# interstellar/zkvm

Hardware: AMD Instinct MI355X
Metric: ZkVM tx verifications/sec (batch) (higher is better)
Workload: dtype u32 limb pairs of radix-2^51 (v_mad_u64_u32)

## Files before the change

zkvm_amd/csrc/kernels.hpp:

```cpp
#pragma once
#include "curve.hpp"
#include "quad.hpp"
#include "sc_dev.hpp"

namespace zk {

constexpr uint32_t ENTRY_NEG = 1u << 31;
constexpr uint32_t ENTRY_DYN = 1u << 30;
constexpr uint32_t ENTRY_IDX = (1u << 30) - 1;
constexpr int NIELS_WORDS = 32;
constexpr int EXT_WORDS = 40;
constexpr int REDUCE_CHUNK = 64;
#ifndef ZK_REDUCE_CHUNK_BIG
#define ZK_REDUCE_CHUNK_BIG 16
#endif
constexpr int REDUCE_CHUNK_BIG = ZK_REDUCE_CHUNK_BIG;
constexpr int TABLE_WORDS = 24;
constexpr int TABLE_STRIDE = 32;

struct JobDesc {
  const uint32_t* dyn_scalars;
  const uint64_t* dyn_offsets;
  uint64_t n_dyn;
  const uint32_t* st_scalars;
  const uint32_t* st_index;
  const uint64_t* st_offsets;
  uint64_t n_static;
  uint32_t n_msm;
  int w;
  int n_windows;
  uint32_t n_buckets;
};


__device__ __forceinline__ void load_niels(ge_niels& q, const uint32_t* row) {
  const uint4* r4 = reinterpret_cast<const uint4*>(row);
  uint32_t w[32];
#pragma unroll
  for (int i = 0; i < 8; ++i) {
    uint4 v = r4[i];
    w[4 * i] = v.x; w[4 * i + 1] = v.y; w[4 * i + 2] = v.z; w[4 * i + 3] = v.w;
  }
#pragma unroll
  for (int i = 0; i < 10; ++i) { q.ypx.v[i] = w[i]; q.ymx.v[i] = w[10 + i]; q.xy2d.v[i] = w[20 + i]; }
}

__device__ __forceinline__ void store_niels(uint32_t* row, const ge_niels& q, uint32_t valid) {
  uint32_t w[32];
#pragma unroll
  for (int i = 0; i < 10; ++i) { w[i] = q.ypx.v[i]; w[10 + i] = q.ymx.v[i]; w[20 + i] = q.xy2d.v[i]; }
  w[30] = valid; w[31] = 0;
  uint4* r4 = reinterpret_cast<uint4*>(row);
#pragma unroll
  for (int i = 0; i < 8; ++i) r4[i] = make_uint4(w[4 * i], w[4 * i + 1], w[4 * i + 2], w[4 * i + 3]);
}

__device__ __forceinline__ void load_ext(ge& p, const uint32_t* row) {
  const uint4* r4 = reinterpret_cast<const uint4*>(row);
  uint32_t w[40];
#pragma unroll
  for (int i = 0; i < 10; ++i) {
    uint4 v = r4[i];
    w[4 * i] = v.x; w[4 * i + 1] = v.y; w[4 * i + 2] = v.z; w[4 * i + 3] = v.w;
  }
#pragma unroll
  for (int i = 0; i < 10; ++i) { p.X.v[i] = w[i]; p.Y.v[i] = w[10 + i]; p.Z.v[i] = w[20 + i]; p.T.v[i] = w[30 + i]; }
}

__device__ __forceinline__ void store_ext(uint32_t* row, const ge& p) {
  uint32_t w[40];
#pragma unroll
  for (int i = 0; i < 10; ++i) { w[i] = p.X.v[i]; w[10 + i] = p.Y.v[i]; w[20 + i] = p.Z.v[i]; w[30 + i] = p.T.v[i]; }
  uint4* r4 = reinterpret_cast<uint4*>(row);
#pragma unroll
  for (int i = 0; i < 10; ++i) r4[i] = make_uint4(w[4 * i], w[4 * i + 1], w[4 * i + 2], w[4 * i + 3]);
}

__device__ __forceinline__ void load_table_row(ge_niels& q, const uint32_t* row) {
  const uint4* r4 = reinterpret_cast<const uint4*>(row);
  uint32_t w[24];
#pragma unroll
  for (int i = 0; i < 6; ++i) {
    uint4 v = r4[i];
    w[4 * i] = v.x; w[4 * i + 1] = v.y; w[4 * i + 2] = v.z; w[4 * i + 3] = v.w;
  }
  fe_from_words(q.ypx, w);
  fe_from_words(q.ymx, w + 8);
  fe_from_words(q.xy2d, w + 16);
}

__device__ __forceinline__ void store_table_row(uint32_t* row, const ge_niels& q) {
  uint32_t w[24];
  fe_to_words(w, q.ypx);
  fe_to_words(w + 8, q.ymx);
  fe_to_words(w + 16, q.xy2d);
  uint4* r4 = reinterpret_cast<uint4*>(row);
#pragma unroll
  for (int i = 0; i < 6; ++i) r4[i] = make_uint4(w[4 * i], w[4 * i + 1], w[4 * i + 2], w[4 * i + 3]);
}

__device__ __forceinline__ uint32_t find_row(const uint64_t* __restrict__ offsets, uint32_t n_msm, uint64_t g) {
  uint32_t lo = 0, hi = n_msm;
  while (hi - lo > 1) {
    uint32_t mid = (lo + hi) >> 1;
    if (offsets[mid] <= g) lo = mid; else hi = mid;
  }
  return lo;
}

__global__ void __launch_bounds__(256)
k_decompress(const uint32_t* __restrict__ pts, uint32_t* __restrict__ rows, uint64_t n,
             const uint64_t* __restrict__ offsets, uint32_t n_msm, uint32_t* __restrict__ msm_fail,
             unsigned long long* __restrict__ bad_index, uint8_t* __restrict__ ok_out) {
  uint64_t i = (uint64_t)blockIdx.x * blockDim.x + threadIdx.x;
  if (i >= n) return;
  const uint4* p4 = reinterpret_cast<const uint4*>(pts + 8 * i);
  uint4 a = p4[0], b = p4[1];
  uint32_t w[8] = {a.x, a.y, a.z, a.w, b.x, b.y, b.z, b.w};
  fe x, y;
  bool ok = ristretto_decode_affine(x, y, w);
  ge_niels q;
  niels_from_affine(q, x, y);
  if (!ok) niels_identity(q);
  if (rows) store_niels(rows + NIELS_WORDS * i, q, ok ? 1u : 0u);
  if (ok_out) ok_out[i] = ok ? 1 : 0;
  if (!ok) {
    if (bad_index) atomicMin(bad_index, (unsigned long long)i);
    if (msm_fail) {
      uint32_t m = (n_msm > 1 && offsets) ? find_row(offsets, n_msm, i) : 0;
      atomicOr(&msm_fail[m], 1u);
    }
  }
}

struct DecodeRoutes {
  uint64_t n[4] = {0, 0, 0, 0};
  void note(bool split, uint64_t points) {
    n[split ? 2 : 0] += 1;
    n[split ? 3 : 1] += points;
  }
};

constexpr int DEC_WORDS = 64;

struct DecFront { fe s, u1, u2, v, w, w7; bool pre_ok; };
__device__ __forceinline__ void dec_front(DecFront& d, const uint32_t* __restrict__ pts, uint64_t i) {
  const uint4* p4 = reinterpret_cast<const uint4*>(pts + 8 * i);
  uint4 a = p4[0], b = p4[1];
  uint32_t w[8] = {a.x, a.y, a.z, a.w, b.x, b.y, b.z, b.w};
  fe ss, u2_sqr, t;
  fe_from_words(d.s, w);
  uint32_t chk[8];
  fe_to_words(chk, d.s);
  bool canonical = true;
#pragma unroll
  for (int k = 0; k < 8; ++k) canonical &= (chk[k] == w[k]);
// ... 872 lines not shown
    accept[m] = failed ? 0 : 1;
    return;
  }
  const bool ident = have ? ge_is_identity(acc) : true;
  accept[m] = (ident && !failed) ? 1 : 0;
}

__global__ void __launch_bounds__(64)
k_from_uniform(const uint32_t* __restrict__ in, uint32_t* __restrict__ out, uint64_t n) {
  const uint64_t i = (uint64_t)blockIdx.x * blockDim.x + threadIdx.x;
  if (i >= n) return;
  uint32_t w[16];
  const uint4* i4 = reinterpret_cast<const uint4*>(in + 16 * i);
#pragma unroll
  for (int k = 0; k < 4; ++k) { uint4 v = i4[k]; w[4 * k] = v.x; w[4 * k + 1] = v.y; w[4 * k + 2] = v.z; w[4 * k + 3] = v.w; }
  ge p;
  ristretto_from_uniform_words(p, w);
  uint32_t enc[8];
  ristretto_encode(enc, p);
  uint4* o = reinterpret_cast<uint4*>(out + 8 * i);
  o[0] = make_uint4(enc[0], enc[1], enc[2], enc[3]);
  o[1] = make_uint4(enc[4], enc[5], enc[6], enc[7]);
}

__global__ void __launch_bounds__(64)
k_spin(unsigned long long cycles, uint32_t* __restrict__ sink) {
  const unsigned long long t0 = clock64();
  unsigned long long spins = 0;
  while ((unsigned long long)clock64() - t0 < cycles) ++spins;
  if (sink && spins == ~0ull) *sink = 1;
}

__global__ void __launch_bounds__(256)
k_hbm_copy(const uint4* __restrict__ src, uint4* __restrict__ dst, uint64_t n_vec) {
  const uint64_t i = (uint64_t)blockIdx.x * 256 + threadIdx.x;
  if (i < n_vec) dst[i] = src[i];
}

__global__ void __launch_bounds__(256)
k_batch_init(uint32_t* __restrict__ status, uint32_t* __restrict__ msm_fail, uint32_t* __restrict__ wellformed,
             uint32_t n_msm) {
  const uint32_t i = blockIdx.x * blockDim.x + threadIdx.x;
  if (i < n_msm) {
    msm_fail[i] = 0;
    if (wellformed) wellformed[i] = 0xffffffffu;
  }
  if (i == 0) {
    status[0] = 0; status[1] = 0;
    status[2] = 0xffffffffu; status[3] = 0xffffffffu;
    status[8] = 0;
    status[9] = 0;
  }
}

__global__ void __launch_bounds__(256)
k_pack_bitmap(const uint8_t* __restrict__ accept, const uint32_t* __restrict__ wellformed ,
              uint8_t* __restrict__ bitmap, uint32_t n_msm) {
  const uint32_t byte = blockIdx.x * blockDim.x + threadIdx.x;
  if (byte >= (n_msm + 7) / 8) return;
  uint32_t v = 0;
#pragma unroll
  for (int k = 0; k < 8; ++k) {
    const uint32_t i = byte * 8 + k;
    if (i < n_msm && accept[i] && (!wellformed || wellformed[i])) v |= 1u << k;
  }
  bitmap[byte] = (uint8_t)v;
}


__global__ void __launch_bounds__(64)
k_tbl_base(const uint32_t* __restrict__ rows , uint32_t* __restrict__ base, uint32_t n_set, int w, int W) {
  const uint32_t j = blockIdx.x * blockDim.x + threadIdx.x;
  if (j >= n_set) return;
  ge_niels q;
  load_niels(q, rows + (uint64_t)j * NIELS_WORDS);
  ge p;
  ge_identity(p);
  ge_madd(p, p, q, false);
  for (int t = 0; t < W; ++t) {
    store_ext(base + ((uint64_t)t * n_set + j) * EXT_WORDS, p);
    if (t + 1 < W) {
      for (int k = 0; k < w - 1; ++k) ge_double<false>(p, p);
      ge_double<true>(p, p);
    }
  }
}

__global__ void __launch_bounds__(64)
k_tbl_multiples(const uint32_t* __restrict__ base, uint32_t* __restrict__ tmp, uint32_t* __restrict__ table,
                uint64_t n_lanes, uint32_t H) {
  const uint64_t lane = (uint64_t)blockIdx.x * blockDim.x + threadIdx.x;
  if (lane >= n_lanes) return;
  ge p, q;
  load_ext(p, base + lane * EXT_WORDS);
  q = p;
  fe prod = fe_one();
  uint32_t* mytmp = tmp + lane * (uint64_t)H * EXT_WORDS;
  for (uint32_t d = 0; d < H; ++d) {
    if (d) ge_add(q, q, p);
    fe_mul(prod, prod, q.Z);
    ge rec;
    rec.X = q.X; rec.Y = q.Y; rec.Z = q.Z; rec.T = prod;
    store_ext(mytmp + (uint64_t)d * EXT_WORDS, rec);
  }
  fe inv;
  fe_invert(inv, prod);
  uint32_t* myrows = table + lane * (uint64_t)H * TABLE_STRIDE;
  for (uint32_t d = H; d-- > 0;) {
    ge rec;
    load_ext(rec, mytmp + (uint64_t)d * EXT_WORDS);
    fe prev = fe_one();
    if (d) {
      ge r2;
      load_ext(r2, mytmp + (uint64_t)(d - 1) * EXT_WORDS);
      prev = r2.T;
    }
    fe zinv, x, y;
    fe_mul(zinv, inv, prev);
    fe_mul(inv, inv, rec.Z);
    fe_mul(x, rec.X, zinv);
    fe_mul(y, rec.Y, zinv);
    ge_niels nq;
    niels_from_affine(nq, x, y);
    store_table_row(myrows + (uint64_t)d * TABLE_STRIDE, nq);
  }
}

__global__ void __launch_bounds__(256)
k_static_digits(const uint32_t* __restrict__ st_scalars, int16_t* __restrict__ digits, uint64_t n_static, int w,
                int W, uint32_t* __restrict__ status, const uint32_t* __restrict__ row_map ,
                const uint32_t* __restrict__ n_active , uint32_t rows_per_msm, uint32_t fold_small_negatives) {
  uint64_t k = (uint64_t)blockIdx.x * blockDim.x + threadIdx.x;
  if (k >= n_static) return;
  if (row_map) {
    const uint32_t slot = (uint32_t)(k / rows_per_msm);
    if (slot >= *n_active) return;
    k = (uint64_t)row_map[slot] * rows_per_msm + k % rows_per_msm;
  }
  const uint32_t* sc = st_scalars + 8 * k;
  if (sc[7] >> 31) atomicOr(&status[0], 2u);
  for (int t = 0; t < W; ++t) digits[(uint64_t)t * n_static + k] = 0;
  if (fold_small_negatives) {
    const uint32_t l[8] = ZK_SC_L;
    uint32_t v[8];
    uint64_t br = 0;
    for (int i = 0; i < 8; ++i) { const uint64_t d = (uint64_t)l[i] - sc[i] - br; v[i] = (uint32_t)d; br = (d >> 32) & 1; }
    uint32_t high = v[0] >> 14;
    for (int i = 1; i < 8; ++i) high |= v[i];
    if (br == 0 && high == 0 && v[0] != 0 && w >= 15) { digits[k] = (int16_t)(-(int)v[0]); return; }
  }
  for_each_digit(sc, w, W, [&](int t, int d) { digits[(uint64_t)t * n_static + k] = (int16_t)d; });
}

template <bool kSkipZeros>
__global__ void __launch_bounds__(256)
k_static_accumulate(const int16_t* __restrict__ digits, const uint64_t* __restrict__ st_offsets,
                    const uint32_t* __restrict__ st_index, const uint32_t* __restrict__ table, uint32_t n_set,
                    uint32_t H, int W, int P, uint32_t n_msm, uint64_t n_static, uint32_t* __restrict__ partials,
                    const uint32_t* __restrict__ row_map ,
                    const uint32_t* __restrict__ n_active ,
                    uint32_t interleave ) {
  const uint64_t lane = (uint64_t)blockIdx.x * blockDim.x + threadIdx.x;
  if (lane >= (uint64_t)n_msm * W * P) return;
  const uint32_t part = (uint32_t)(lane % P);
  uint32_t slot = (uint32_t)((lane / P) % n_msm);
  const uint32_t t = (uint32_t)(lane / ((uint64_t)P * n_msm));
  if (n_active && slot >= *n_active) return;
  if (interleave > 1) { const uint32_t per = n_msm / interleave; slot = (slot % per) * interleave + slot / per; }
  const uint32_t tx = row_map ? row_map[slot] : slot;
  const uint64_t k0 = st_offsets[tx], k1 = st_offsets[tx + 1];
  const int16_t* dig = digits + (uint64_t)t * n_static;
  const uint64_t tbase = (uint64_t)t * n_set;
  ge acc;
  ge_identity(acc);
  auto fetch = [&](uint64_t k, ge_niels& q, bool& neg, bool& any) {
    int d = dig[k];
    d = (d == -32768) ? 32768 : d;
    any = d != 0;
    const uint32_t idx = st_index ? st_index[k] : (uint32_t)(k - k0);
    const uint32_t mag = (uint32_t)(d < 0 ? -d : d);
    if (!kSkipZeros || any) load_table_row(q, table + ((tbase + idx) * H + (mag ? mag - 1 : 0)) * TABLE_STRIDE);
    if (!any) niels_identity(q);
    neg = d < 0;
  };
  uint64_t k = k0 + part;
  ge_niels cur, nxt;
  bool cur_neg = false, nxt_neg = false, cur_any = false, nxt_any = false;
  if (k < k1) fetch(k, cur, cur_neg, cur_any);
  while (k < k1) {
    const uint64_t kn = k + P;
    if (kn < k1) fetch(kn, nxt, nxt_neg, nxt_any);
    if (!kSkipZeros || __any(cur_any)) ge_madd(acc, acc, cur, cur_neg);
    cur = nxt; cur_neg = nxt_neg; cur_any = nxt_any;
    k = kn;
  }
  store_ext(partials + (((uint64_t)slot * W + t) * P + part) * EXT_WORDS, acc);
}

__device__ inline void static_combine_slot(const uint32_t* __restrict__ partials, uint32_t n_partials, const uint32_t* __restrict__ dyn_sum,
                                           const uint8_t* __restrict__ dyn_ok, uint32_t slot, uint32_t tx, int lane,
                                           uint8_t* __restrict__ accept, uint32_t* __restrict__ out_points) {
  ge acc;
  ge_identity(acc);
  for (uint32_t c = lane; c < n_partials; c += 64) {
    ge p;
    load_ext(p, partials + ((uint64_t)slot * n_partials + c) * EXT_WORDS);
    ge_add(acc, acc, p);
  }
  if (lane == 0 && dyn_sum) {
    ge p;
    load_ext(p, dyn_sum + (uint64_t)tx * EXT_WORDS);
    ge_add(acc, acc, p);
  }
#pragma unroll 1
  for (int delta = 32; delta >= 1; delta >>= 1) {
    ge other;
    shfl_down_ge(other, acc, delta);
    if (lane < delta) ge_add(acc, acc, other);
  }
  if (lane == 0) {
    accept[tx] = (ge_is_identity(acc) && (!dyn_ok || dyn_ok[tx])) ? 1 : 0;
    if (out_points) store_ext(out_points + (uint64_t)slot * EXT_WORDS, acc);
  }
}

constexpr uint32_t COMBINE_LANES = 8;

__global__ void __launch_bounds__(64)
k_static_combine(const uint32_t* __restrict__ partials, uint32_t n_partials, const uint32_t* __restrict__ dyn_sum,
                 const uint8_t* __restrict__ dyn_ok, const uint32_t* __restrict__ row_map,
                 const uint32_t* __restrict__ n_active, uint32_t n_slots, uint8_t* __restrict__ accept,
                 uint32_t* __restrict__ out_points ) {
  const uint32_t n = n_active ? min(*n_active, n_slots) : n_slots;
  const uint32_t g = blockIdx.x * 64 + threadIdx.x, sub = g % COMBINE_LANES, first = (blockIdx.x * 64) / COMBINE_LANES;
  if (first >= n) return;
  const uint32_t mine = g / COMBINE_LANES, slot = mine < n ? mine : n - 1;
  const uint32_t tx = row_map ? row_map[slot] : slot;
  ge acc;
  ge_identity(acc);
  for (uint32_t c = sub; c < n_partials; c += COMBINE_LANES) {
    ge p;
    load_ext(p, partials + ((uint64_t)slot * n_partials + c) * EXT_WORDS);
    ge_add(acc, acc, p);
  }
  if (sub == 0 && dyn_sum) {
    ge p;
    load_ext(p, dyn_sum + (uint64_t)tx * EXT_WORDS);
    ge_add(acc, acc, p);
  }
#pragma unroll 1
  for (int delta = COMBINE_LANES / 2; delta >= 1; delta >>= 1) {
    ge other;
    shfl_down_ge(other, acc, delta);
    if (sub < (uint32_t)delta) ge_add(acc, acc, other);
  }
  if (sub == 0 && mine < n) {
    accept[tx] = (ge_is_identity(acc) && (!dyn_ok || dyn_ok[tx])) ? 1 : 0;
    if (out_points) store_ext(out_points + (uint64_t)slot * EXT_WORDS, acc);
  }
}

__device__ inline void static_row_share(ge& acc, const int16_t* __restrict__ digits, uint64_t n_static_total, uint64_t k0, uint32_t ns,
                                        const uint32_t* __restrict__ st_index, const uint32_t* __restrict__ table, uint32_t n_set,
                                        uint32_t H, int W, uint32_t tid, uint32_t n_threads) {
  ge_identity(acc);
  const uint32_t items = (uint32_t)W * ns;
  auto fetch = [&](uint32_t i, ge_niels& q, bool& neg) {
    const uint32_t t = i / ns, j = i - t * ns;
    const uint64_t k = k0 + j;
    int d = digits[(uint64_t)t * n_static_total + k];
    d = (d == -32768) ? 32768 : d;
    const uint32_t idx = st_index ? st_index[k] : j;
    const uint32_t mag = (uint32_t)(d < 0 ? -d : d);
    load_table_row(q, table + (((uint64_t)t * n_set + idx) * H + (mag ? mag - 1 : 0)) * TABLE_STRIDE);
    if (d == 0) niels_identity(q);
    neg = d < 0;
  };
  uint32_t i = tid;
  ge_niels cur, nxt;
  bool cur_neg = false, nxt_neg = false;
  if (i < items) fetch(i, cur, cur_neg);
  while (i < items) {
    const uint32_t in = i + n_threads;
    if (in < items) fetch(in, nxt, nxt_neg);
    ge_madd(acc, acc, cur, cur_neg);
    cur = nxt; cur_neg = nxt_neg;
    i = in;
  }
}

__global__ void __launch_bounds__(512)
k_recheck_fused(const int16_t* __restrict__ digits, const uint64_t* __restrict__ st_offsets, const uint32_t* __restrict__ st_index,
                const uint32_t* __restrict__ table, uint32_t n_set, uint32_t H, int W, uint64_t n_static_total,
                uint32_t* __restrict__ partials , const uint32_t* __restrict__ dyn_sum,
                const uint8_t* __restrict__ dyn_ok, const uint32_t* __restrict__ row_map, const uint32_t* __restrict__ n_active,
                uint8_t* __restrict__ accept, uint32_t* __restrict__ out_points) {
  const uint32_t slot = blockIdx.x;
  if (slot >= *n_active) return;
  const uint32_t tx = row_map[slot];
  const uint64_t k0 = st_offsets[tx];
  ge acc;
  static_row_share(acc, digits, n_static_total, k0, (uint32_t)(st_offsets[tx + 1] - k0), st_index, table, n_set, H, W, threadIdx.x, blockDim.x);
  store_ext(partials + ((uint64_t)slot * blockDim.x + threadIdx.x) * EXT_WORDS, acc);
  __threadfence_block();
  __syncthreads();
  if (threadIdx.x < 64) static_combine_slot(partials, blockDim.x, dyn_sum, dyn_ok, slot, tx, (int)threadIdx.x, accept, out_points);
}

__global__ void __launch_bounds__(64)
k_static_values(const uint32_t* __restrict__ partials, uint32_t n_partials, uint32_t* __restrict__ out_enc) {
  const uint32_t m = blockIdx.x;
  const int lane = threadIdx.x;
  ge acc;
  ge_identity(acc);
  for (uint32_t c = lane; c < n_partials; c += 64) {
    ge p;
    load_ext(p, partials + ((uint64_t)m * n_partials + c) * EXT_WORDS);
    ge_add(acc, acc, p);
  }
#pragma unroll 1
  for (int delta = 32; delta >= 1; delta >>= 1) {
    ge other;
    shfl_down_ge(other, acc, delta);
    if (lane < delta) ge_add(acc, acc, other);
  }
  if (lane == 0) {
    uint32_t enc[8];
    ristretto_encode(enc, acc);
    uint4* o = reinterpret_cast<uint4*>(out_enc + 8 * (uint64_t)m);
    o[0] = make_uint4(enc[0], enc[1], enc[2], enc[3]);
    o[1] = make_uint4(enc[4], enc[5], enc[6], enc[7]);
  }
}

constexpr uint32_t ROW_SUM_LANES = 8;
__global__ void __launch_bounds__(64)
k_static_row_sums(const uint32_t* __restrict__ partials, uint32_t n_partials, uint32_t n_rows, uint32_t* __restrict__ out_ext) {
  const uint32_t g = blockIdx.x * 64 + threadIdx.x, sub = g % ROW_SUM_LANES;
  const uint32_t row = g / ROW_SUM_LANES, m = row < n_rows ? row : n_rows - 1;
  ge acc;
  ge_identity(acc);
  for (uint32_t c = sub; c < n_partials; c += ROW_SUM_LANES) {
    ge p;
    load_ext(p, partials + ((uint64_t)m * n_partials + c) * EXT_WORDS);
    ge_add(acc, acc, p);
  }
#pragma unroll 1
  for (int delta = ROW_SUM_LANES / 2; delta >= 1; delta >>= 1) {
    ge other;
// ... 401 lines not shown
```

zkvm_amd/csrc/pipe_plan.hpp:

```cpp
#pragma once
#include <algorithm>
#include <cstddef>
#include <cstdint>

namespace zk {

constexpr int PLAN_EXT_WORDS = 40, PLAN_NIELS_WORDS = 32, PLAN_SMALL_TBL = 8;
constexpr int TAIL_THREADS = 512;
constexpr size_t LOCATE_MIN_BATCH = 2048;

constexpr uint64_t FILL_LANES = 131072, MAX_PARTS = 16;
inline int static_parts(uint64_t B, int W, int forced) {
  return forced > 0 ? forced : (int)std::max<uint64_t>(1, std::min<uint64_t>(MAX_PARTS, (FILL_LANES + B * W - 1) / (B * W)));
}
inline uint64_t static_lanes_room(uint64_t B, int W, int forced) {
  return forced > 0 ? B * W * forced : std::min<uint64_t>(MAX_PARTS * B * W, FILL_LANES - 1 + B * W);
}
constexpr uint64_t MAX_ROW_PARTS = 64;
inline int row_parts(uint64_t rows, int W) {
  const uint64_t cells = std::max<uint64_t>(rows * W, 1);
  return (int)std::max<uint64_t>(1, std::min<uint64_t>(MAX_ROW_PARTS, (FILL_LANES + cells - 1) / cells));
}
inline uint64_t row_lanes_room(uint64_t rows, int W) { return std::min<uint64_t>(MAX_ROW_PARTS * rows * W, FILL_LANES - 1 + rows * W); }
inline int group_parts(uint64_t rows, int W) { return (int)std::max<uint64_t>(1, std::min<uint64_t>(32, (65536 + rows * W - 1) / (rows * W))); }

struct SmallWindowBytes { size_t dyn_rows, window_sums, window_flags, msm_fail, small_tbl, recoded; };
inline SmallWindowBytes small_window_bytes(uint64_t B, uint64_t n_dyn) {
  const uint64_t pts = std::max<uint64_t>(n_dyn, 1), ext = PLAN_EXT_WORDS * 4;
  return {(size_t)(pts * PLAN_NIELS_WORDS * 4), (size_t)(B * 64 * ext), (size_t)(B * 64 * 4), (size_t)(B * 4), (size_t)(pts * PLAN_SMALL_TBL * ext),
          (size_t)(pts * 32)};
}

struct PipeShape { uint64_t n_msm, n_dyn, n_static; int W; bool whole_proof; uint32_t ns; };
struct PipeKnobs { int group_size, locate_mode, locate_parts, forced_parts; bool want_reasons; };

struct PipePlan {
  size_t nbytes;
  int P; uint64_t n_lanes;
  uint32_t group, n_groups;
  bool locate, spec;
  uint32_t grp_rows;
  int Pg, Pf, Pl;
  size_t grp_sc, grp_digits, grp_partials, grp_ok, row_map, grp_fail, grp_fail_sum, grp_ws, grp_wf, grp_dyn, rechk_pts;
  size_t accept, accept2, bitmap, pinned, status, digits, st_partials, dynsum;
  SmallWindowBytes small;
};

inline PipePlan plan_pipe(const PipeShape& sh, const PipeKnobs& k) {
  PipePlan p = {};
  const size_t B = (size_t)sh.n_msm, ext = (size_t)PLAN_EXT_WORDS * 4;
  const int W = sh.W;
  p.nbytes = (B + 7) / 8;
  p.P = static_parts(B, W, k.forced_parts);
  p.n_lanes = (uint64_t)B * W * p.P;
  p.group = (sh.whole_proof && k.group_size > 1) ? (uint32_t)std::min<size_t>((size_t)k.group_size, B) : 1;
  p.n_groups = (uint32_t)((B + p.group - 1) / p.group);
  p.locate = p.group > 1 && (k.locate_mode >= 2 || (k.locate_mode == 0 && B >= LOCATE_MIN_BATCH));
  p.spec = p.locate && k.locate_mode == 3;
  p.grp_rows = p.spec ? 2 * p.n_groups : p.n_groups;
  p.Pg = 1; p.Pf = 32;
  p.Pl = k.locate_parts > 0 ? k.locate_parts : 32;
  if (p.group > 1) {
    const size_t rows = p.grp_rows, ns = sh.ns, groups = p.n_groups;
    p.Pg = group_parts(rows, W);
    p.grp_sc = rows * ns * 32; p.grp_digits = rows * ns * W * 2;
    p.grp_partials = rows * std::max<size_t>((size_t)W * std::max(p.Pg, p.locate && !p.spec ? p.Pl : 0), TAIL_THREADS) * ext;
    p.grp_ok = groups; p.grp_fail = groups * 12; p.grp_fail_sum = p.grp_dyn = groups * ext;
    p.grp_ws = groups * 64 * ext; p.grp_wf = groups * 64 * 4;
    p.row_map = B * 4; p.rechk_pts = B * ext;
  }
  p.accept = p.accept2 = B; p.bitmap = p.nbytes; p.status = 64;
  p.pinned = p.nbytes + 64 + (k.want_reasons ? B : 0);
  p.digits = (size_t)(std::max<uint64_t>(sh.n_static, 1) * W * 2);
  p.st_partials = (size_t)(std::max<uint64_t>(static_lanes_room(B, W, k.forced_parts), p.group > 1 ? (uint64_t)B * std::max(W * p.Pf, TAIL_THREADS) : 0) * ext);
  p.dynsum = B * ext;
  p.small = small_window_bytes(B, sh.n_dyn);
  return p;
}

}
```

zkvm_amd/csrc/zkgpu.hip:

```cpp
#include "../../include/zkgpu.h"
#include "../../include/zkgpu_hooks.h"
#include "kernels.hpp"
#include "keccak.hpp"

#include <hip/hip_runtime.h>

#include <algorithm>
#include <chrono>
#include <cerrno>
#include <cstdio>
#include <cstring>
#include <functional>
#include <memory>
#include <mutex>
#include <string>
#include <map>
#include <atomic>
#include <dirent.h>
#include <sys/random.h>
#include <unistd.h>
#include <thread>
#include <type_traits>
#include <vector>

// ... 411 lines not shown
  }
  TRY(ensure(c, c->bin_order, rt.bin_order));
  {
    Launch l(c, "k_bin_order");
    if (!part_sort)
      hipLaunchKernelGGL(k_bin_classes, dim3(blocks_for(n_bins, 256)), dim3(256), 0, s, (const uint32_t*)c->bins.p, n_bins,
                         class_count);
    hipLaunchKernelGGL(k_class_scan, dim3(1), dim3(256), 0, s, (const uint32_t*)class_count, class_cursor);
    hipLaunchKernelGGL(k_bin_order, dim3(blocks_for(n_bins, 256)), dim3(256), 0, s, (const uint32_t*)c->bins.p, n_bins,
                       class_cursor, (uint32_t*)c->bin_order.p, heavy, fat, fat_cap);
  }
  if (decompress_aside) HIP_TRY(c, hipStreamWaitEvent(s, c->ev_join, 0));
  {
    const unsigned fat_blocks = rt.fat_blocks;
    Launch l(c, "k_bucket_accumulate");
    hipLaunchKernelGGL(k_bucket_accumulate, dim3(fat_blocks + blocks_for(n_bins, 256)), dim3(256), 0, s,
                       (const uint32_t*)c->bins.p, (const uint32_t*)c->entries.p, job.d_static_rows,
                       (const uint32_t*)c->dyn_rows.p, (uint32_t*)c->buckets.p, n_bins,
                       (const uint32_t*)c->bin_order.p, (const uint32_t*)fat, fat_cap, fat_blocks);
  }
  {
    Launch l(c, "k_bucket_heavy");
    hipLaunchKernelGGL(k_bucket_heavy, dim3(512), dim3(256), 0, s, (const uint32_t*)c->bins.p,
                       (const uint32_t*)c->entries.p, job.d_static_rows, (const uint32_t*)c->dyn_rows.p,
                       (uint32_t*)c->buckets.p, (const uint32_t*)heavy);
  }
  uint32_t* partials = chunks == 1 ? (uint32_t*)c->window_sums.p : (uint32_t*)c->partials.p;
  uint32_t* pflags = chunks == 1 ? (uint32_t*)c->window_flags.p : (uint32_t*)c->partial_flags.p;
  {
    Launch l(c, "k_bucket_reduce");
    c->msm_routes[rt.quad_reduce ? zkgpu_ctx::RT_QUAD_REDUCE : zkgpu_ctx::RT_LANE_REDUCE] += 1;
    if (rt.quad_reduce)
      hipLaunchKernelGGL(k_bucket_reduce_quad, dim3(blocks_for(4 * n_tasks, 256)), dim3(256), 0, s, (const uint32_t*)c->bins.p,
                         (const uint32_t*)c->buckets.p, partials, pflags, n_tasks, jd.n_buckets, chunks, chunk_size);
    else
      hipLaunchKernelGGL(k_bucket_reduce, dim3(blocks_for(n_tasks, 256)), dim3(256), 0, s, (const uint32_t*)c->bins.p,
                         (const uint32_t*)c->buckets.p, partials, pflags, n_tasks, jd.n_buckets, chunks, chunk_size);
  }
  if (rt.window_partials) {
    c->msm_routes[zkgpu_ctx::RT_WINDOW_PARTIALS] += 1;
    Launch l(c, "k_window_partials");
    hipLaunchKernelGGL(k_window_partials, dim3((unsigned)n_wins), dim3(256), 0, s, (const uint32_t*)c->partials.p,
                       (const uint32_t*)c->partial_flags.p, (uint32_t*)c->window_sums.p,
                       (uint32_t*)c->window_flags.p, chunks);
  }
  HIP_TRY(c, hipGetLastError());
  return ZKGPU_OK;
}

int msm_device(zkgpu_ctx* c, const void* d_scalars, const void* d_points, size_t n, uint8_t out[32],
               size_t* bad_index) {
  memset(out, 0, 32);
  if (bad_index) *bad_index = (size_t)-1;
  if (n == 0) return ZKGPU_OK;
  Job job;
  job.d_dyn_scalars = (const uint32_t*)d_scalars;
  job.d_dyn_points = (const uint32_t*)d_points;
  job.n_dyn = n;
  job.n_msm = 1;
  JobDesc jd;
  TRY(run_to_windows(c, job, jd));
  const size_t W = (size_t)jd.n_windows;
  const size_t bytes = W * EXT_WORDS * 4 + W * 4 + 64;
  TRY(ensure_pinned(c, bytes));
  char* h = (char*)c->pinned;
  HIP_TRY(c, hipMemcpyAsync(h, c->window_sums.p, W * EXT_WORDS * 4, hipMemcpyDeviceToHost, c->stream));
  HIP_TRY(c, hipMemcpyAsync(h + W * EXT_WORDS * 4, c->window_flags.p, W * 4, hipMemcpyDeviceToHost, c->stream));
  HIP_TRY(c, hipMemcpyAsync(h + W * EXT_WORDS * 4 + W * 4, c->status.p, 16, hipMemcpyDeviceToHost, c->stream));
  HIP_TRY(c, hipStreamSynchronize(c->stream));
  if (c->profiling) prof_collect(c);
  const uint32_t* hs = (const uint32_t*)(h + W * EXT_WORDS * 4 + W * 4);
  unsigned long long bad;
  memcpy(&bad, hs + 2, 8);
  if (bad != ~0ull) {
    if (bad_index) *bad_index = (size_t)bad;
    return ZKGPU_EINVALID_POINT;
  }
  if (hs[0] & 2u) { c->last_error = "scalar with bit 255 set"; return ZKGPU_EINVAL; }
  const uint32_t* sums = (const uint32_t*)h;
  const uint32_t* flags = (const uint32_t*)(h + W * EXT_WORDS * 4);
  ge acc;
  bool have = false;
  for (int t = (int)W - 1; t >= 0; --t) {
    if (have) {
      for (int k = 0; k < jd.w - 1; ++k) ge_double<false>(acc, acc);
      ge_double<true>(acc, acc);
    }
    if (flags[t]) {
      ge p;
      const uint32_t* r = sums + (size_t)t * EXT_WORDS;
      for (int i = 0; i < 10; ++i) { p.X.v[i] = r[i]; p.Y.v[i] = r[10 + i]; p.Z.v[i] = r[20 + i]; p.T.v[i] = r[30 + i]; }
      if (have) ge_add(acc, acc, p); else { acc = p; have = true; }
    }
  }
  if (!have) return ZKGPU_OK;
  uint32_t enc[8];
  ristretto_encode(enc, acc);
  memcpy(out, enc, 32);
  return ZKGPU_OK;
}

int small_msm_launch(zkgpu_ctx* c, const Job& job, hipStream_t st);
int tx_reasons_enqueue(zkgpu_ctx* c, const uint32_t* d_wellformed, size_t B, hipStream_t st, char* h_out);
int tx_reasons_parked(zkgpu_ctx* c, const uint32_t* d_wellformed, size_t B, int rc);

int small_window_workspace(zkgpu_ctx* c, const SmallWindowBytes& b, bool with_tables) {
  TRY(ensure(c, c->dyn_rows, b.dyn_rows));
  TRY(ensure(c, c->window_sums, b.window_sums));
  TRY(ensure(c, c->window_flags, b.window_flags));
  TRY(ensure(c, c->msm_fail, b.msm_fail));
  if (with_tables) TRY(ensure(c, c->small_tbl, b.small_tbl));
  return with_tables ? ensure(c, c->recoded, b.recoded) : ZKGPU_OK;
}

uint32_t* n_recheck_dev(zkgpu_ctx* c) { return (uint32_t*)((char*)c->status.p + 32); }
uint32_t* n_fail_dev(zkgpu_ctx* c) { return (uint32_t*)((char*)c->status.p + 36); }

void batch_init_launch(zkgpu_ctx* c, hipStream_t s, size_t B, bool with_wellformed) {
  Launch l(c, "k_batch_init", s);
  hipLaunchKernelGGL(k_batch_init, dim3(blocks_for(B, 256)), dim3(256), 0, s, (uint32_t*)c->status.p, (uint32_t*)c->msm_fail.p,
                     with_wellformed ? (uint32_t*)c->prep_wf.p : (uint32_t*)nullptr, (uint32_t)B);
}

enum class Horner { ACCEPT_ONLY, VALUES, SUMS, GROUP_SUMS };
void msm_finish_launch(zkgpu_ctx* c, hipStream_t s, size_t n, int w, int n_windows, Horner what, const uint32_t* failed_of = nullptr, uint32_t group = 0) {
  const bool groups = what == Horner::GROUP_SUMS;
  Launch l(c, "k_msm_finish_quad", s);
  hipLaunchKernelGGL(k_msm_finish_quad, dim3(blocks_for(4 * (uint64_t)n, 256)), dim3(256), 0, s,
                     (const uint32_t*)(groups ? c->grp_ws.p : c->window_sums.p), (const uint32_t*)(groups ? c->grp_wf.p : c->window_flags.p),
                     groups ? (const uint32_t*)nullptr : (const uint32_t*)c->msm_fail.p, groups ? (uint8_t*)nullptr : (uint8_t*)c->accept.p,
                     what == Horner::VALUES ? (uint32_t*)c->values.p : (uint32_t*)nullptr,
                     groups ? (uint32_t*)c->grp_dyn.p : what == Horner::SUMS ? (uint32_t*)c->dynsum.p : (uint32_t*)nullptr, (uint32_t)n, w,
                     n_windows, failed_of, group);
}

void pack_bitmap_launch(zkgpu_ctx* c, hipStream_t s, size_t B, const Buffer& accept, const uint32_t* d_wellformed) {
  Launch l(c, "k_pack_bitmap", s);
  hipLaunchKernelGGL(k_pack_bitmap, dim3(blocks_for((B + 7) / 8, 256)), dim3(256), 0, s, (const uint8_t*)accept.p, d_wellformed,
                     (uint8_t*)c->bitmap.p, (uint32_t)B);
}

struct RowQueue { const uint32_t* row_map = nullptr; const uint32_t* n_rows_dev = nullptr; };

void static_digits_launch(zkgpu_ctx* c, hipStream_t s, const zkgpu_pointset* ps, const uint32_t* d_scalars, uint64_t n, RowQueue q = {},
                          uint32_t ns = 0, uint32_t fold = 0) {
  Launch l(c, "k_static_digits", s);
  hipLaunchKernelGGL(k_static_digits, dim3(blocks_for(n, 256)), dim3(256), 0, s, d_scalars, (int16_t*)c->digits.p, n, ps->tbl_w,
                     ps->tbl_W, (uint32_t*)c->status.p, q.row_map, q.n_rows_dev, ns, fold);
}

struct StaticRows { uint32_t rows; uint64_t n_terms; int parts; const Buffer* digits; const Buffer* partials; RowQueue queue = {}; };
void static_accumulate_launch(zkgpu_ctx* c, hipStream_t s, const zkgpu_pointset* ps, const uint64_t* d_offsets, const uint32_t* d_index,
                              const StaticRows& r, uint32_t kinds = 1, bool skip_zeros = false) {
  Launch l(c, "k_static_accumulate", s);
  hipLaunchKernelGGL(skip_zeros ? k_static_accumulate<true> : k_static_accumulate<false>,
                     dim3(blocks_for((uint64_t)r.rows * ps->tbl_W * r.parts, 256)), dim3(256), 0, s, (const int16_t*)r.digits->p,
                     d_offsets, d_index, (const uint32_t*)ps->table, (uint32_t)ps->n, ps->tbl_H, ps->tbl_W, r.parts, r.rows, r.n_terms,
                     (uint32_t*)r.partials->p, r.queue.row_map, r.queue.n_rows_dev, kinds);
}

void static_combine_launch(zkgpu_ctx* c, hipStream_t s, size_t B, int lanes, bool with_dyn, RowQueue q = {}) {
  Launch l(c, "k_static_combine", s);
  hipLaunchKernelGGL(k_static_combine, dim3(blocks_for((uint64_t)B * COMBINE_LANES, 64)), dim3(64), 0, s, (const uint32_t*)c->st_partials.p,
                     (uint32_t)lanes, with_dyn ? (const uint32_t*)c->dynsum.p : (const uint32_t*)nullptr,
                     with_dyn ? (const uint8_t*)c->accept.p : (const uint8_t*)nullptr, q.row_map, q.n_rows_dev, (uint32_t)B,
                     (uint8_t*)c->accept2.p, q.row_map ? (uint32_t*)c->rechk_pts.p : (uint32_t*)nullptr);
}

void recheck_fused_launch(zkgpu_ctx* c, hipStream_t s, const zkgpu_pointset* ps, const Job& job, uint32_t rows, bool keep_sums) {
  Launch l(c, "k_recheck_fused", s);
  hipLaunchKernelGGL(k_recheck_fused, dim3(rows), dim3(TAIL_THREADS), 0, s, (const int16_t*)c->digits.p, job.d_st_offsets, job.d_st_index,
                     (const uint32_t*)ps->table, (uint32_t)ps->n, ps->tbl_H, ps->tbl_W, (uint64_t)job.n_static, (uint32_t*)c->st_partials.p,
                     (const uint32_t*)c->dynsum.p, (const uint8_t*)c->accept.p, (const uint32_t*)c->row_map.p,
                     (const uint32_t*)n_recheck_dev(c), (uint8_t*)c->accept2.p, keep_sums ? (uint32_t*)c->rechk_pts.p : (uint32_t*)nullptr);
}

int results_enqueue(zkgpu_ctx* c, hipStream_t s, size_t nbytes, size_t status_bytes) {
  HIP_TRY(c, hipGetLastError());
  HIP_TRY(c, hipMemcpyAsync(c->pinned, c->bitmap.p, nbytes, hipMemcpyDeviceToHost, s));
  HIP_TRY(c, hipMemcpyAsync((char*)c->pinned + nbytes, c->status.p, status_bytes, hipMemcpyDeviceToHost, s));
  return ZKGPU_OK;
}

void mark_pending(zkgpu_ctx* c, size_t B) { c->pending = true; c->pending_batch = B; c->sync_result_valid = false; }

int batch_device_enqueue(zkgpu_ctx* c, const Job& job, bool values) {
  const size_t B = job.n_msm, nbytes = (B + 7) / 8;
  c->split = zkgpu_ctx::SplitOp{1, B, values, c->stream};
  if (B == 0) return ZKGPU_OK;
  JobDesc jd;
  if (plan_msm(MsmShape{job.n_msm, job.n_dyn, job.n_static, job.max_dyn_row, c->forced_w, MSM_BATCH}).small) {
    hipStream_t s = c->stream;
    jd.w = 4; jd.n_windows = 64;
    c->last_w = 4;
    TRY(small_window_workspace(c, small_window_bytes(B, job.n_dyn), false));
    TRY(ensure(c, c->status, 64));
    batch_init_launch(c, s, B, false);
    decompress_launch(c, job, s);
    TRY(small_msm_launch(c, job, s));
  } else {
    TRY(run_to_windows(c, job, jd));
  }
  TRY(ensure(c, c->accept, B));
  TRY(ensure(c, c->bitmap, nbytes));
  TRY(ensure_pinned(c, nbytes + 64 + (values ? 32 * B : 0)));
  if (values) TRY(ensure(c, c->values, 32 * B));
  msm_finish_launch(c, c->stream, B, jd.w, jd.n_windows, values ? Horner::VALUES : Horner::ACCEPT_ONLY);
  pack_bitmap_launch(c, c->stream, B, c->accept, job.d_wellformed);
  TRY(results_enqueue(c, c->stream, nbytes, 16));
  if (values) HIP_TRY(c, hipMemcpyAsync((char*)c->pinned + nbytes + 64, c->values.p, 32 * B, hipMemcpyDeviceToHost, c->stream));
  return ZKGPU_OK;
}

int batch_collect(zkgpu_ctx* c, uint8_t* accept_bitmap, uint8_t* values) {
  const zkgpu_ctx::SplitOp op = c->split;
  c->split = zkgpu_ctx::SplitOp{};
  const size_t B = op.batch, nbytes = (B + 7) / 8;
  memset(accept_bitmap, 0, nbytes);
  if (values) memset(values, 0, 32 * B);
  if (op.kind == 0) return ZKGPU_EINVAL;
  if (B == 0) return ZKGPU_OK;
  HIP_TRY(c, hipStreamSynchronize(op.stream));
  if (c->profiling) prof_collect(c);
  const char* h = (const char*)c->pinned;
  uint32_t st;
  memcpy(&st, h + nbytes, 4);
  if (st & 2u) { c->last_error = "scalar with bit 255 set"; return ZKGPU_EINVAL; }
  memcpy(accept_bitmap, h, nbytes);
  if (values && op.values) memcpy(values, h + nbytes + 64, 32 * B);
  return ZKGPU_OK;
}

int batch_device(zkgpu_ctx* c, const Job& job, uint8_t* accept_bitmap, uint8_t* values = nullptr) {
  const size_t B = job.n_msm;
  memset(accept_bitmap, 0, (B + 7) / 8);
  if (values) memset(values, 0, 32 * B);
  const int rc = batch_device_enqueue(c, job, values != nullptr);
  if (rc != ZKGPU_OK) { c->split = zkgpu_ctx::SplitOp{}; return rc; }
  return batch_collect(c, accept_bitmap, values);
}

int small_tables_launch(zkgpu_ctx* c, const uint32_t* d_scalars, uint64_t n_dyn, hipStream_t st) {
  TRY(ensure(c, c->small_tbl, std::max<uint64_t>(n_dyn, 1) * SMALL_TBL * EXT_WORDS * 4));
  TRY(ensure(c, c->recoded, std::max<uint64_t>(n_dyn, 1) * 32));
  Launch l(c, "k_small_tables", st);
  hipLaunchKernelGGL(k_small_tables, dim3(blocks_for(n_dyn, 64)), dim3(64), 0, st, d_scalars,
                     (const uint32_t*)c->dyn_rows.p, n_dyn, (uint32_t*)c->small_tbl.p, (uint32_t*)c->recoded.p,
                     (uint32_t*)c->status.p);
  return ZKGPU_OK;
}

int small_accumulate_launch(zkgpu_ctx* c, const Job& job, hipStream_t st) {
  const size_t B = job.n_msm;
  Launch l(c, "k_small_accumulate", st);
  const int parts = small_parts(B);
  c->msm_routes[zkgpu_ctx::RT_SMALL] += 1;
  c->msm_routes[zkgpu_ctx::RT_SMALL_PARTS] = (uint64_t)parts;
  hipLaunchKernelGGL(k_small_accumulate, dim3((unsigned)B), dim3(64 * parts), (size_t)(parts - 1) * 41 * 64 * 4, st,
                     (const uint32_t*)c->recoded.p, job.d_dyn_offsets, (const uint32_t*)c->small_tbl.p, (uint32_t)B,
                     (uint32_t*)c->window_sums.p, (uint32_t*)c->window_flags.p);
  return ZKGPU_OK;
}

int small_msm_launch(zkgpu_ctx* c, const Job& job, hipStream_t st) {
  TRY(small_tables_launch(c, job.d_dyn_scalars, job.n_dyn, st));
  return small_accumulate_launch(c, job, st);
}

int batch_device_tables_enqueue(zkgpu_ctx* c, const Job& job, const zkgpu_pointset* ps) {
  const size_t B = job.n_msm, nbytes = (B + 7) / 8;
  c->split = zkgpu_ctx::SplitOp{2, B, false, c->stream};
  if (B == 0) return ZKGPU_OK;
  hipStream_t s = c->stream, s2 = c->stream2;
  const bool has_dyn = job.n_dyn > 0;
  const int W = ps->tbl_W;
  const int P = static_parts(B, W, c->forced_parts);
  const uint64_t n_lanes = (uint64_t)B * W * P;
  TRY(ensure(c, c->accept, B));
  TRY(ensure(c, c->accept2, B));
  TRY(ensure(c, c->bitmap, nbytes));
  TRY(ensure_pinned(c, nbytes + 64));
  TRY(ensure(c, c->status, 64));
  TRY(ensure(c, c->digits, std::max<uint64_t>(job.n_static, 1) * W * 2));
  TRY(ensure(c, c->st_partials, n_lanes * EXT_WORDS * 4));
  TRY(ensure(c, c->dynsum, B * EXT_WORDS * 4));
  HIP_TRY(c, hipMemsetAsync(c->status.p, 0, 8, s));
  HIP_TRY(c, hipMemsetAsync((char*)c->status.p + 8, 0xff, 8, s));
  HIP_TRY(c, hipEventRecord(c->ev_fork, s));
  HIP_TRY(c, hipStreamWaitEvent(s2, c->ev_fork, 0));
  if (has_dyn) {
    Job dj = job;
    dj.d_st_scalars = nullptr; dj.d_st_index = nullptr; dj.d_st_offsets = nullptr; dj.n_static = 0;
    JobDesc jd;
    const bool small = plan_msm(MsmShape{job.n_msm, job.n_dyn, job.n_static, job.max_dyn_row, c->forced_w, MSM_TABLES}).small;
    c->msm_routes[small ? zkgpu_ctx::RT_TABLES_SMALL : zkgpu_ctx::RT_TABLES_BUCKET] += 1;
    if (small) {
      jd.w = 4; jd.n_windows = 64;
      c->last_w = 4;
      TRY(small_window_workspace(c, small_window_bytes(B, job.n_dyn), false));
      HIP_TRY(c, hipMemsetAsync(c->msm_fail.p, 0, (size_t)B * 4, s));
      decompress_launch(c, job, s);
      TRY(small_msm_launch(c, job, s));
    } else {
      TRY(run_to_windows(c, dj, jd, false));
    }
    msm_finish_launch(c, s, B, jd.w, jd.n_windows, Horner::SUMS);
  }
  if (job.n_static) static_digits_launch(c, s2, ps, job.d_st_scalars, job.n_static);
  static_accumulate_launch(c, s2, ps, job.d_st_offsets, job.d_st_index, {(uint32_t)B, job.n_static, P, &c->digits, &c->st_partials});
  HIP_TRY(c, hipEventRecord(c->ev_join, s2));
// ... 2645 lines not shown
```

Baseline: 3.383 million.

## Split static accumulate lanes across multiple waves with LDS reduction

When the static-accumulate launch has too few wavefronts to fill the chip, each logical lane is spread over S waves in one workgroup. Each wave walks a strided subset of terms, then the sub-waves write their extended points to LDS and wave 0 adds them before storing the partial. This targets low occupancy and long serial chains on small batches. The cost is extra LDS traffic, a barrier, S-1 extra point additions per lane, and possibly larger LDS allocations that need a raised attribute.

```diff
diff --git a/zkvm_amd/csrc/kernels.hpp b/zkvm_amd/csrc/kernels.hpp
--- a/zkvm_amd/csrc/kernels.hpp
+++ b/zkvm_amd/csrc/kernels.hpp
@@ -1,7 +1,9 @@
 #pragma once
+#include <atomic>
 #include "curve.hpp"
 #include "quad.hpp"
 #include "sc_dev.hpp"
+#include "pipe_plan.hpp"
 
 namespace zk {
 
@@ -1180,49 +1182,103 @@
   for_each_digit(sc, w, W, [&](int t, int d) { digits[(uint64_t)t * n_static + k] = (int16_t)d; });
 }
 
-template <bool kSkipZeros>
-__global__ void __launch_bounds__(256)
+template <bool kSkipZeros, bool kSplit>
+__global__ void __launch_bounds__(kSplit ? 64 * MAX_STATIC_SPLIT : 256)
 k_static_accumulate(const int16_t* __restrict__ digits, const uint64_t* __restrict__ st_offsets,
                     const uint32_t* __restrict__ st_index, const uint32_t* __restrict__ table, uint32_t n_set,
                     uint32_t H, int W, int P, uint32_t n_msm, uint64_t n_static, uint32_t* __restrict__ partials,
                     const uint32_t* __restrict__ row_map ,
                     const uint32_t* __restrict__ n_active ,
                     uint32_t interleave ) {
-  const uint64_t lane = (uint64_t)blockIdx.x * blockDim.x + threadIdx.x;
-  if (lane >= (uint64_t)n_msm * W * P) return;
+  const uint32_t S = kSplit ? blockDim.x >> 6 : 1u;
+  const uint32_t sub = kSplit ? (uint32_t)__builtin_amdgcn_readfirstlane((int)(threadIdx.x >> 6)) : 0u;
+  const uint64_t lane = kSplit ? (uint64_t)blockIdx.x * 64 + (threadIdx.x & 63) : (uint64_t)blockIdx.x * blockDim.x + threadIdx.x;
+  bool live = lane < (uint64_t)n_msm * W * P;
   const uint32_t part = (uint32_t)(lane % P);
   uint32_t slot = (uint32_t)((lane / P) % n_msm);
   const uint32_t t = (uint32_t)(lane / ((uint64_t)P * n_msm));
-  if (n_active && slot >= *n_active) return;
-  if (interleave > 1) { const uint32_t per = n_msm / interleave; slot = (slot % per) * interleave + slot / per; }
-  const uint32_t tx = row_map ? row_map[slot] : slot;
-  const uint64_t k0 = st_offsets[tx], k1 = st_offsets[tx + 1];
-  const int16_t* dig = digits + (uint64_t)t * n_static;
-  const uint64_t tbase = (uint64_t)t * n_set;
+  if (live && n_active && slot >= *n_active) live = false;
+  if (!kSplit && !live) return;
   ge acc;
   ge_identity(acc);
-  auto fetch = [&](uint64_t k, ge_niels& q, bool& neg, bool& any) {
-    int d = dig[k];
-    d = (d == -32768) ? 32768 : d;
-    any = d != 0;
-    const uint32_t idx = st_index ? st_index[k] : (uint32_t)(k - k0);
-    const uint32_t mag = (uint32_t)(d < 0 ? -d : d);
-    if (!kSkipZeros || any) load_table_row(q, table + ((tbase + idx) * H + (mag ? mag - 1 : 0)) * TABLE_STRIDE);
-    if (!any) niels_identity(q);
-    neg = d < 0;
-  };
-  uint64_t k = k0 + part;
-  ge_niels cur, nxt;
-  bool cur_neg = false, nxt_neg = false, cur_any = false, nxt_any = false;
-  if (k < k1) fetch(k, cur, cur_neg, cur_any);
-  while (k < k1) {
-    const uint64_t kn = k + P;
-    if (kn < k1) fetch(kn, nxt, nxt_neg, nxt_any);
-    if (!kSkipZeros || __any(cur_any)) ge_madd(acc, acc, cur, cur_neg);
-    cur = nxt; cur_neg = nxt_neg; cur_any = nxt_any;
-    k = kn;
+  bool set = false;
+  if (live) {
+    if (interleave > 1) { const uint32_t per = n_msm / interleave; slot = (slot % per) * interleave + slot / per; }
+    const uint32_t tx = row_map ? row_map[slot] : slot;
+    const uint64_t k0 = st_offsets[tx], k1 = st_offsets[tx + 1];
+    const int16_t* dig = digits + (uint64_t)t * n_static;
+    const uint64_t tbase = (uint64_t)t * n_set;
+    auto fetch = [&](uint64_t k, ge_niels& q, bool& neg, bool& any) {
+      int d = dig[k];
+      d = (d == -32768) ? 32768 : d;
+      any = d != 0;
+      const uint32_t idx = st_index ? st_index[k] : (uint32_t)(k - k0);
+      const uint32_t mag = (uint32_t)(d < 0 ? -d : d);
+      if (!kSkipZeros || any) load_table_row(q, table + ((tbase + idx) * H + (mag ? mag - 1 : 0)) * TABLE_STRIDE);
+      if (!any) niels_identity(q);
+      neg = d < 0;
+    };
+    const uint64_t step = (uint64_t)P * S;
+    uint64_t k = k0 + part + (uint64_t)P * sub;
+    ge_niels cur, nxt;
+    bool cur_neg = false, nxt_neg = false, cur_any = false, nxt_any = false;
+    set = k < k1;
+    if (k < k1) fetch(k, cur, cur_neg, cur_any);
+    while (k < k1) {
+      const uint64_t kn = k + step;
+      if (kn < k1) fetch(kn, nxt, nxt_neg, nxt_any);
+      if (!kSkipZeros || __any(cur_any)) ge_madd(acc, acc, cur, cur_neg);
+      cur = nxt; cur_neg = nxt_neg; cur_any = nxt_any;
+      k = kn;
+    }
+  }
+  if constexpr (kSplit) {
+    extern __shared__ __attribute__((aligned(16))) uint32_t smem[];
+    const uint32_t l = threadIdx.x & 63;
+    if (sub > 0) {
+      uint32_t* mine = smem + (sub - 1) * STATIC_SPLIT_SLOT_WORDS;
+      mine[40 * 64 + l] = set ? 1u : 0u;
+      if (set) {
+#pragma unroll
+        for (int q = 0; q < 10; ++q) {
+          mine[q * 64 + l] = acc.X.v[q]; mine[(10 + q) * 64 + l] = acc.Y.v[q];
+          mine[(20 + q) * 64 + l] = acc.Z.v[q]; mine[(30 + q) * 64 + l] = acc.T.v[q];
+        }
+      }
+    }
+    __syncthreads();
+    if (sub != 0 || !live) return;
+#pragma unroll 1
+    for (uint32_t o = 1; o < S; ++o) {
+      const uint32_t* theirs = smem + (o - 1) * STATIC_SPLIT_SLOT_WORDS;
+      if (theirs[40 * 64 + l]) {
+        ge other;
+#pragma unroll
+        for (int q = 0; q < 10; ++q) {
+          other.X.v[q] = theirs[q * 64 + l]; other.Y.v[q] = theirs[(10 + q) * 64 + l];
+          other.Z.v[q] = theirs[(20 + q) * 64 + l]; other.T.v[q] = theirs[(30 + q) * 64 + l];
+        }
+        ge_add(acc, acc, other);
+      }
+    }
   }
   store_ext(partials + (((uint64_t)slot * W + t) * P + part) * EXT_WORDS, acc);
+}
+
+using StaticAccumulateKernel = decltype(&k_static_accumulate<false, false>);
+inline StaticAccumulateKernel static_accumulate_kernel(bool skip_zeros, uint32_t S, int device) {
+  if (S == 1) return skip_zeros ? k_static_accumulate<true, false> : k_static_accumulate<false, false>;
+  if (static_split_lds_bytes(S) > 64 * 1024) {
+    static std::atomic<uint64_t> announced{0};
+    const uint64_t bit = 1ull << (device & 63);
+    if (!(announced.load(std::memory_order_relaxed) & bit)) {
+      const int bytes = (int)static_split_lds_bytes(MAX_STATIC_SPLIT);
+      (void)hipFuncSetAttribute((const void*)k_static_accumulate<false, true>, hipFuncAttributeMaxDynamicSharedMemorySize, bytes);
+      (void)hipFuncSetAttribute((const void*)k_static_accumulate<true, true>, hipFuncAttributeMaxDynamicSharedMemorySize, bytes);
+      announced.fetch_or(bit, std::memory_order_relaxed);
+    }
+  }
+  return skip_zeros ? k_static_accumulate<true, true> : k_static_accumulate<false, true>;
 }
 
 __device__ inline void static_combine_slot(const uint32_t* __restrict__ partials, uint32_t n_partials, const uint32_t* __restrict__ dyn_sum,
diff --git a/zkvm_amd/csrc/pipe_plan.hpp b/zkvm_amd/csrc/pipe_plan.hpp
--- a/zkvm_amd/csrc/pipe_plan.hpp
+++ b/zkvm_amd/csrc/pipe_plan.hpp
@@ -23,6 +23,23 @@
 }
 inline uint64_t row_lanes_room(uint64_t rows, int W) { return std::min<uint64_t>(MAX_ROW_PARTS * rows * W, FILL_LANES - 1 + rows * W); }
 inline int group_parts(uint64_t rows, int W) { return (int)std::max<uint64_t>(1, std::min<uint64_t>(32, (65536 + rows * W - 1) / (rows * W))); }
+
+constexpr uint64_t CHIP_SIMDS = 1024;
+constexpr uint64_t STATIC_SPLIT_TARGET = 4;
+constexpr uint32_t MAX_STATIC_SPLIT = 8;
+constexpr uint32_t STATIC_SPLIT_SLOT_WORDS = 41 * 64;
+constexpr uint32_t static_split(uint64_t lanes) {
+  const uint64_t waves = lanes > 64 ? (lanes + 63) / 64 : 1;
+  uint32_t s = 1;
+  while (s < MAX_STATIC_SPLIT && waves * s < STATIC_SPLIT_TARGET * CHIP_SIMDS) s *= 2;
+  return s;
+}
+constexpr size_t static_split_lds_bytes(uint32_t s) { return (size_t)(s - 1) * STATIC_SPLIT_SLOT_WORDS * 4; }
+static_assert(static_split(STATIC_SPLIT_TARGET * CHIP_SIMDS * 64) == 1 && static_split(STATIC_SPLIT_TARGET * CHIP_SIMDS * 64 - 64) == 2 &&
+              static_split(~0ull >> 8) == 1, "a launch that already gives every SIMD its share is not split");
+static_assert(static_split(640 * 19 * 6) == 4, "the group launch of a benched device batch (10 240 payments over 14-bit tables)");
+static_assert(static_split(1) == MAX_STATIC_SPLIT && static_split(0) == MAX_STATIC_SPLIT, "few lanes: the cap");
+static_assert((MAX_STATIC_SPLIT & (MAX_STATIC_SPLIT - 1)) == 0 && MAX_STATIC_SPLIT <= 8 && 64 * MAX_STATIC_SPLIT <= 1024, "a power of two, one workgroup");
 
 struct SmallWindowBytes { size_t dyn_rows, window_sums, window_flags, msm_fail, small_tbl, recoded; };
 inline SmallWindowBytes small_window_bytes(uint64_t B, uint64_t n_dyn) {
diff --git a/zkvm_amd/csrc/zkgpu.hip b/zkvm_amd/csrc/zkgpu.hip
--- a/zkvm_amd/csrc/zkgpu.hip
+++ b/zkvm_amd/csrc/zkgpu.hip
@@ -587,10 +587,10 @@
 struct StaticRows { uint32_t rows; uint64_t n_terms; int parts; const Buffer* digits; const Buffer* partials; RowQueue queue = {}; };
 void static_accumulate_launch(zkgpu_ctx* c, hipStream_t s, const zkgpu_pointset* ps, const uint64_t* d_offsets, const uint32_t* d_index,
                               const StaticRows& r, uint32_t kinds = 1, bool skip_zeros = false) {
+  const uint64_t lanes = (uint64_t)r.rows * ps->tbl_W * r.parts; const uint32_t S = static_split(lanes);
   Launch l(c, "k_static_accumulate", s);
-  hipLaunchKernelGGL(skip_zeros ? k_static_accumulate<true> : k_static_accumulate<false>,
-                     dim3(blocks_for((uint64_t)r.rows * ps->tbl_W * r.parts, 256)), dim3(256), 0, s, (const int16_t*)r.digits->p,
-                     d_offsets, d_index, (const uint32_t*)ps->table, (uint32_t)ps->n, ps->tbl_H, ps->tbl_W, r.parts, r.rows, r.n_terms,
+  hipLaunchKernelGGL(static_accumulate_kernel(skip_zeros, S, c->device), dim3(blocks_for(lanes, S > 1 ? 64 : 256)), dim3(S > 1 ? 64 * S : 256), static_split_lds_bytes(S), s,
+                     (const int16_t*)r.digits->p, d_offsets, d_index, (const uint32_t*)ps->table, (uint32_t)ps->n, ps->tbl_H, ps->tbl_W, r.parts, r.rows, r.n_terms,
                      (uint32_t*)r.partials->p, r.queue.row_map, r.queue.n_rows_dev, kinds);
 }
 
```

Result: no change. 3.368 million (median of 2 runs) (-0.5%).
